# AniketRajpoot/DeepMusicGeneration

Hardware: NVIDIA B200
Metric: generated_tokens_per_sec (higher is better)
Workload: dtype bf16

## Files before the change

### deepmusicgeneration_b200/csrc/attention_decode2.cu

```cuda
#include "attention_decode3.cuh"

namespace dmg {

bool attn_decode2_supported(int Dh, int M) { return Dh == 64 && M >= 64 && M % 64 == 0 && d2_pick_groups(M) > 0; }

template <int G>
__global__ void __launch_bounds__((4 * G + 1) * 32, 1)
attn_decode2_kernel(const __grid_constant__ CUtensorMap tmK, const __grid_constant__ CUtensorMap tmV,
                    const __grid_constant__ CUtensorMap tmR, const AttnDecodeArgs a, int n_stages, int b0) {
  extern __shared__ __align__(1024) uint8_t d2_smem[];
  attn_decode2_body<G>(tmK, tmV, tmR, a, n_stages, b0, (int)blockIdx.x, (int)gridDim.x, d2_smem);
}

template <int G>
static int launch_d2(const TensorMap2D* tmK, const TensorMap2D* tmV, const TensorMap2D* tmR, const AttnDecodeArgs& a, int b0,
                     int num_sms, cudaStream_t st) {
  const int ns = d2_pick_stages(a.M, G);
  const D2Layout L = d2_layout(a.M, G, ns);
  static int configured = 0;
  if (configured < L.total) {
    DMG_CUDA_OK(cudaFuncSetAttribute(attn_decode2_kernel<G>, cudaFuncAttributeMaxDynamicSharedMemorySize, L.total));
    configured = L.total;
  }
  DMG_CHECK(ns >= 2, "attn_decode2: no stage count fits (M=%d)", a.M);
  const long long NI = (long long)a.B * a.H;
  const int grid = (int)(NI < num_sms ? NI : num_sms);
  return launch_k(attn_decode2_kernel<G>, dim3(grid), dim3((4 * G + 1) * 32), L.total, st, 1, *(const CUtensorMap*)tmK->bytes,
                  *(const CUtensorMap*)tmV->bytes, *(const CUtensorMap*)tmR->bytes, a, ns, b0);
}

bool attn_decode3_supported(int Dh, int M) { return Dh == 64 && M >= D3_KEYS && M <= 512 && M % D3_KEYS == 0 && d3_pick_stages(M) >= 2; }

__global__ void __launch_bounds__(D3_THREADS, 1)
attn_decode3_kernel(const __grid_constant__ CUtensorMap tmK, const __grid_constant__ CUtensorMap tmV,
                    const __grid_constant__ CUtensorMap tmR, const AttnDecodeArgs a, int n_stages, int b0) {
  extern __shared__ __align__(1024) uint8_t d3_smem[];
  attn_decode3_body<D3_TEAMS>(tmK, tmV, tmR, a, n_stages, b0, (int)blockIdx.x, (int)gridDim.x, d3_smem);
}

static int attn_decode3(const TensorMap2D* tmK, const TensorMap2D* tmV, const TensorMap2D* tmR, const AttnDecodeArgs& a_in, int b0,
                        int num_sms, cudaStream_t st) {
  const int ns = d3_pick_stages(a_in.M);
  const D3Layout L = d3_layout(a_in.M, ns);
  static int configured = 0;
  if (configured < L.total) {
    DMG_CUDA_OK(cudaFuncSetAttribute(attn_decode3_kernel, cudaFuncAttributeMaxDynamicSharedMemorySize, L.total));
    configured = L.total;
  }
  const int HD = a_in.H * 64;
  const int per = (int)((long long)D3_CAP * num_sms / a_in.H);
  DMG_CHECK(per >= 1, "attn_decode3: %d heads do not fit %d CTAs of %d items", a_in.H, num_sms, D3_CAP);
  for (int c0 = 0; c0 < a_in.B; c0 += per) {
    AttnDecodeArgs a = a_in;
    a.B = a_in.B - c0 < per ? a_in.B - c0 : per;
    a.qkv = a_in.qkv + (size_t)c0 * 3 * HD;
    a.out = a_in.out + (size_t)c0 * HD;
    a.kring = a_in.kring + (size_t)c0 * a_in.H * a_in.M * 64;
    a.vring = a_in.vring + (size_t)c0 * a_in.H * a_in.M * 64;
    const long long NI = (long long)a.B * a.H;
    const int grid = (int)(NI < num_sms ? NI : num_sms);
    if (launch_k(attn_decode3_kernel, dim3(grid), dim3(D3_THREADS), L.total, st, 1, *(const CUtensorMap*)tmK->bytes,
                 *(const CUtensorMap*)tmV->bytes, *(const CUtensorMap*)tmR->bytes, a, ns, b0 + c0)) return -1;
  }
  return 0;
}

int attn_decode2(const TensorMap2D* tmK, const TensorMap2D* tmV, const TensorMap2D* tmR, const AttnDecodeArgs& a_in, int b0,
                 int num_sms, cudaStream_t st) {
  static const int no_early = getenv("DMG_NO_EARLY_KV") ? 1 : 0;
  static const int env_v2 = getenv("DMG_ATTN_DECODE_V2") ? 1 : 0;
  AttnDecodeArgs a = a_in;
  a.no_early_kv = no_early;
  DMG_CHECK(a.Dcap >= a.M + 1, "attn_decode2: rel-pos cache too small (%d < %d)", a.Dcap, a.M + 1);
  if (!a.force_v2 && !env_v2 && attn_decode3_supported(64, a.M))
    return attn_decode3(tmK, tmV, tmR, a, b0, num_sms, st);
  const int G = d2_pick_groups(a.M);
  DMG_CHECK(G > 0, "attn_decode2: mem_len %d not supported", a.M);
  if (G == 4) return launch_d2<4>(tmK, tmV, tmR, a, b0, num_sms, st);
  if (G == 2) return launch_d2<2>(tmK, tmV, tmR, a, b0, num_sms, st);
  return launch_d2<1>(tmK, tmV, tmR, a, b0, num_sms, st);
}

}
```

### deepmusicgeneration_b200/csrc/attention_decode3.cuh

```cuda
#pragma once
#include "attention_decode2.cuh"

namespace dmg {

constexpr int D3_TEAMS = 2;
constexpr int D3_CAP = 16;
constexpr int D3_KEYS = 128;
constexpr int D3_TILE = D3_KEYS * 128;
constexpr int D3_THREADS = D3_TEAMS * 5 * 32;

struct D3Layout {
  int r_boxes, n_stages, tab_stride, free_bytes;
  int off_ring, off_r, off_tab, off_team, team_bytes, off_bar, total;
};

__host__ __device__ inline D3Layout d3_layout(int M, int n_stages, int teams = D3_TEAMS) {
  D3Layout L;
  L.r_boxes = (M + 1 + 63) / 64;
  L.n_stages = n_stages;
  L.tab_stride = M + 4;
  const int ring = teams * n_stages * D3_TILE;
  L.off_ring = 0;
  L.off_r = ring - L.r_boxes * 8192;
  L.free_bytes = L.off_r;
  L.off_tab = ring;
  L.off_team = L.off_tab + D3_CAP * L.tab_stride * 4;
  L.team_bytes = 2 * 768 + (((M + 16) * 2 + 15) & ~15) + 64;
  L.off_bar = (L.off_team + teams * L.team_bytes + 15) & ~15;
  L.total = L.off_bar + (teams * (2 * n_stages + 4) + 2) * 8 + 1024 ;
  return L;
}

static inline int d3_pick_stages(int M, int teams = D3_TEAMS) {
  for (int s = 6; s >= 2; s--) {
    const D3Layout L = d3_layout(M, s, teams);
    if (L.off_r >= 0 && L.total <= 227 * 1024) return s;
  }
  return 0;
}

template <int T>
__device__ __forceinline__ void attn_decode3_body(const CUtensorMap& tmK, const CUtensorMap& tmV, const CUtensorMap& tmR, const AttnDecodeArgs& a,
                                                  int n_stages, int b0, int cta, int ncta, uint8_t* d3_smem) {
  constexpr int CW = 4 * T;
  uint8_t* base = d3_smem + ((1024u - (smem_u32(d3_smem) & 1023u)) & 1023u);
  const int M = a.M, H = a.H, B = a.B, HD = H * 64;
  const D3Layout L = d3_layout(M, n_stages, T);
  uint8_t* Rres = base + L.off_r;
  float* tab = (float*)(base + L.off_tab);
  const int S = L.tab_stride;
  uint64_t* bars = (uint64_t*)(base + L.off_bar);
  uint64_t* r_full = bars;
  uint64_t* prologue_done = bars + 1;

  const int tid = threadIdx.x, warp = tid >> 5, lane = tid & 31;
  const int nT = M / D3_KEYS;
  pdl_launch_dependents();
  const long long NI = (long long)B * H;
  const int lo = (int)(NI * cta / ncta), hi = (int)(NI * (cta + 1) / ncta);
  const int n_items = hi - lo;

  if (tid == 0) {
    for (int t = 0; t < T; t++) {
      uint64_t* tb = bars + 2 + t * (2 * n_stages + 4);
      for (int s = 0; s < n_stages; s++) {
        mbar_init(&tb[s], 1);
        mbar_init(&tb[n_stages + s], 4);
      }
      for (int s = 0; s < 2; s++) {
        mbar_init(&tb[2 * n_stages + s], 1);
        mbar_init(&tb[2 * n_stages + 2 + s], 4);
      }
    }
    mbar_init(r_full, 1);
    mbar_init(prologue_done, CW);
    mbar_fence_init();
    tma_prefetch_desc(&tmK);
    tma_prefetch_desc(&tmV);
    tma_prefetch_desc(&tmR);
    if (n_items > 0) {
      mbar_expect_tx(r_full, (uint32_t)(L.r_boxes * 8192));
      for (int bx = 0; bx < L.r_boxes; bx++) tma_load_2d(Rres + bx * 8192, &tmR, 0, (lo / B) * a.Dcap + bx * 64, r_full);
    }
  }
  named_bar_sync(4, (CW + T) * 32);

  if (warp >= CW) {
    if (lane == 0) {
      const int team = warp - CW;
      uint64_t* tb = bars + 2 + team * (2 * n_stages + 4);
      uint64_t *full = tb, *empty = tb + n_stages, *q_full = tb + 2 * n_stages, *q_empty = q_full + 2;
      uint8_t* ring = base + L.off_ring;
      float* qbuf = (float*)(base + L.off_team + team * L.team_bytes);
      int s = 0, use = 0, pre = 0;
      bool alias_ok = false;
      const uint64_t kv_policy = l2_policy_evict_first();
      if (team < n_items && !a.no_early_kv) {
        const int it = lo + team, h = it / B, b = it - h * B;
        const int row0 = ((b0 + b) * H + h) * M;
        while (pre < 2 * nT && s < n_stages && (s * T + team + 1) * D3_TILE <= L.free_bytes) {
          mbar_expect_tx(&full[s], (uint32_t)D3_TILE);
          uint8_t* dst = ring + (s * T + team) * D3_TILE;
          const CUtensorMap* tm = pre < nT ? &tmK : &tmV;
          const int r0 = row0 + (pre < nT ? pre : pre - nT) * D3_KEYS;
          tma_load_2d_hint(dst, tm, 0, r0, &full[s], kv_policy);
          tma_load_2d_hint(dst + 8192, tm, 0, r0 + 64, &full[s], kv_policy);
          ++pre; ++s;
        }
        if (s == n_stages) { s = 0; use = 1; }
      }
      pdl_wait();
      for (int i = team, k = 0; i < n_items; i += T, ++k) {
        const int it = lo + i, h = it / B, b = it - h * B;
        const int qs = k & 1;
        mbar_wait(&q_empty[qs], (uint32_t)(((k >> 1) & 1) ^ 1));
        mbar_expect_tx(&q_full[qs], 768);
        const float* qrow = a.qkv + (size_t)b * 3 * HD + h * 64;
        bulk_g2s(qbuf + qs * 192, qrow, 256, &q_full[qs]);
        bulk_g2s(qbuf + qs * 192 + 64, qrow + HD, 256, &q_full[qs]);
        bulk_g2s(qbuf + qs * 192 + 128, qrow + 2 * HD, 256, &q_full[qs]);
        const int row0 = ((b0 + b) * H + h) * M;
        for (int t = (k == 0 ? pre : 0); t < 2 * nT; ++t) {
          if (!alias_ok && (s * T + team + 1) * D3_TILE > L.free_bytes) {
            mbar_wait(prologue_done, 0);
            alias_ok = true;
          }
          mbar_wait(&empty[s], (uint32_t)((use & 1) ^ 1));
          mbar_expect_tx(&full[s], (uint32_t)D3_TILE);
          uint8_t* dst = ring + (s * T + team) * D3_TILE;
          const CUtensorMap* tm = t < nT ? &tmK : &tmV;
          const int r0 = row0 + (t < nT ? t : t - nT) * D3_KEYS;
          tma_load_2d_hint(dst, tm, 0, r0, &full[s], kv_policy);
          tma_load_2d_hint(dst + 8192, tm, 0, r0 + 64, &full[s], kv_policy);
          if (++s == n_stages) { s = 0; ++use; }
        }
      }
    }
    return;
  }

  if (a.dbg && cta == 0 && tid == 0) { unsigned long long t; asm volatile("mov.u64 %0, %%globaltimer;" : "=l"(t)); a.dbg[48] = t; }
#ifdef D2_PROFILE
  long long prof[6] = {0, 0, 0, 0, 0, 0}, sec[8] = {0, 0, 0, 0, 0, 0, 0, 0};
  const long long t_begin = clock64();
  long long t_last = t_begin;
#endif
  pdl_wait();
  const int pos_total = a.dev_state[0], mc = a.dev_state[1];
  const int head = pos_total % M;
  const int team = warp >> 2, w = warp & 3;
  const int g = lane >> 2, t4 = lane & 3;
  const int hi16 = lane >> 4;
  const float sscale = a.scale * D2_LOG2E;

  {
    const uint32_t r_base = smem_u32(Rres);
    const int nblk = (M + 1 + 15) / 16;
    int seg = 0, r_epoch = 0;
    while (seg < n_items) {
      const int h = (lo + seg) / B;
      const int seg_end = min(n_items, (h + 1) * B - lo);
      mbar_wait(r_full, (uint32_t)(r_epoch & 1));
      r_epoch++;
      uint32_t qvf[2][4][2];
#pragma unroll
      for (int nb = 0; nb < 2; nb++) {
        const int item = min(seg + 8 * nb + g, seg_end - 1);
        const float* qrow = a.qkv + (size_t)(lo + item - h * B) * 3 * HD + h * 64;
#pragma unroll
        for (int ks = 0; ks < 4; ks++) {
#pragma unroll
          for (int hh = 0; hh < 2; hh++) {
            const int d = ks * 16 + 2 * t4 + 8 * hh;
            const float2 qq = *(const float2*)(qrow + d), vv = *(const float2*)(a.v + h * 64 + d);
            qvf[nb][ks][hh] = pack_bf16x2(qq.x + vv.x, qq.y + vv.y);
          }
        }
      }
      const bool two = seg_end - seg > 8;
      for (int blk = warp; blk < nblk; blk += CW) {
        const int dr = 16 * blk + (lane & 15);
        const uint32_t r_row = r_base + dr * 128;
        const int rsw = dr & 7;
        float acc0[4] = {0.f, 0.f, 0.f, 0.f}, acc1[4] = {0.f, 0.f, 0.f, 0.f};
#pragma unroll
        for (int ks = 0; ks < 4; ks++) {
          uint32_t c0, c1, c2, c3;
          ldmatrix_x4(r_row + (((2 * ks + hi16) ^ rsw) << 4), c0, c1, c2, c3);
          mma_bf16_16816(acc0, c0, c1, c2, c3, qvf[0][ks][0], qvf[0][ks][1]);
          if (two) mma_bf16_16816(acc1, c0, c1, c2, c3, qvf[1][ks][0], qvf[1][ks][1]);
        }
        const int d0 = 16 * blk + g, d1 = d0 + 8;
#pragma unroll
        for (int nb = 0; nb < 2; nb++) {
          const float* acc = nb ? acc1 : acc0;
          const int i0 = seg + 8 * nb + 2 * t4;
          if (i0 < seg_end) {
            if (d0 <= M) tab[i0 * S + d0] = acc[0];
            if (d1 <= M) tab[i0 * S + d1] = acc[2];
          }
          if (i0 + 1 < seg_end) {
            if (d0 <= M) tab[(i0 + 1) * S + d0] = acc[1];
            if (d1 <= M) tab[(i0 + 1) * S + d1] = acc[3];
          }
        }
      }
      seg = seg_end;
      named_bar_sync(5, CW * 32);
      if (seg < n_items && tid == 0) {
        mbar_expect_tx(r_full, (uint32_t)(L.r_boxes * 8192));
        for (int bx = 0; bx < L.r_boxes; bx++) tma_load_2d(Rres + bx * 8192, &tmR, 0, ((lo + seg) / B) * a.Dcap + bx * 64, r_full);
// ... 160 lines not shown
```

### deepmusicgeneration_b200/csrc/decode_layer.cu

```cuda
#include <cuda.h>

#include "attention_decode3.cuh"
#include "kernels.cuh"
#include "launch.cuh"

namespace dmg {
namespace {

constexpr int DL_STAGES = 10;
constexpr int DL_STAGE = 128 * 128;
constexpr int DL_B_BYTES = DL_ROWS * 128;
constexpr int DL_D = 512;
constexpr int DL_XA_BYTES = DL_ROWS * DL_D * 2;
constexpr int DL_HS_KB = 4;
constexpr int DL_HS_BYTES = DL_HS_KB * DL_B_BYTES;
constexpr int DL_OWN = DL_ROWS / DL_CLUSTER;
constexpr int DL_X1_BYTES = DL_OWN * DL_D * 4;
constexpr int DL_MMAW = 2;
constexpr int DL_THREADS = 32 * (1 + DL_MMAW + 8);
constexpr int DL_EPI0 = 32 * (1 + DL_MMAW);
constexpr int DL_EPI = 256;
constexpr int DL_LN_BYTES = 4 * DL_D * 4;
constexpr int DL_SMEM = DL_STAGES * DL_STAGE + DL_XA_BYTES + DL_HS_BYTES + DL_X1_BYTES + DL_LN_BYTES + 512  + 1024 ;
constexpr int DL_TMEM_COLS = 512;
constexpr int DL_CHAIN = DL_ROWS;
static_assert(DL_SMEM <= 227 * 1024, "decode_layer_kernel: shared memory budget");

__device__ __forceinline__ uint64_t dl_desc_sw128(uint32_t smem_addr) {
  return (uint64_t)((smem_addr & 0x3FFFFu) >> 4) | (1ull << 16) | (64ull << 32) | (1ull << 46) | (2ull << 61);
}
__host__ __device__ constexpr uint32_t dl_idesc(int M, int N) {
  return (1u << 4) | (1u << 7) | (1u << 10) | ((uint32_t)(N >> 3) << 17) | ((uint32_t)(M >> 4) << 24);
}
__device__ __forceinline__ uint32_t dl_cluster_ctarank() {
  uint32_t r;
  asm volatile("mov.u32 %0, %%cluster_ctarank;" : "=r"(r));
  return r;
}
__device__ __forceinline__ void dl_arrive() { asm volatile("barrier.cluster.arrive.release;" ::: "memory"); }
__device__ __forceinline__ void dl_wait() { asm volatile("barrier.cluster.wait.acquire;" ::: "memory"); }
__device__ __forceinline__ void dl_fence_async_all() { asm volatile("fence.proxy.async;" ::: "memory"); }
__device__ __forceinline__ void dl_fence_async_smem() { asm volatile("fence.proxy.async.shared::cta;" ::: "memory"); }

__device__ __forceinline__ void tmem_ld_32x16(uint32_t taddr, uint32_t (&r)[16]) {
  asm volatile(
      "tcgen05.ld.sync.aligned.32x32b.x16.b32 {%0,%1,%2,%3,%4,%5,%6,%7,%8,%9,%10,%11,%12,%13,%14,%15}, [%16];"
      : "=r"(r[0]), "=r"(r[1]), "=r"(r[2]), "=r"(r[3]), "=r"(r[4]), "=r"(r[5]), "=r"(r[6]), "=r"(r[7]), "=r"(r[8]),
        "=r"(r[9]), "=r"(r[10]), "=r"(r[11]), "=r"(r[12]), "=r"(r[13]), "=r"(r[14]), "=r"(r[15])
      : "r"(taddr)
      : "memory");
}
__device__ __forceinline__ void dl_spin(uint64_t* bar, uint32_t parity) {
  uint32_t n = 0;
  while (!mbar_try_wait(bar, parity))
    if (++n > (1u << 27)) __trap();
}
__device__ __forceinline__ float4 ldcg4(const float* p) { return __ldcg((const float4*)p); }
__device__ __forceinline__ void dl_mark(unsigned long long* dbg, int role, int mark) {
  if (dbg == nullptr) return;
  unsigned long long t;
  asm volatile("mov.u64 %0, %%globaltimer;" : "=l"(t));
  dbg[role * 16 + mark] = t;
}

__device__ __forceinline__ float dl_gelu(float x) {
  float t;
  asm("tanh.approx.f32 %0, %1;" : "=f"(t) : "f"(0.7978845608028654f * (x + 0.044715f * x * x * x)));
  return 0.5f * x * (1.f + t);
}

__device__ __forceinline__ void dl_layernorm(float (&z)[64], const float* __restrict__ w, const float* __restrict__ b, int t) {
  float s = 0.f;
#pragma unroll
  for (int i = 0; i < 64; i++) s += z[i];
  s += __shfl_xor_sync(0xffffffffu, s, 1); s += __shfl_xor_sync(0xffffffffu, s, 2); s += __shfl_xor_sync(0xffffffffu, s, 4);
  const float mean = s * (1.f / DL_D);
  float q = 0.f;
#pragma unroll
  for (int i = 0; i < 64; i++) { const float c = z[i] - mean; q += c * c; }
  q += __shfl_xor_sync(0xffffffffu, q, 1); q += __shfl_xor_sync(0xffffffffu, q, 2); q += __shfl_xor_sync(0xffffffffu, q, 4);
  const float rstd = rsqrtf(q * (1.f / DL_D) + 1e-5f);
#pragma unroll
  for (int kb = 0; kb < 8; kb++) {
    const int c = 64 * kb + 8 * t;
    const float4 w0 = *(const float4*)(w + c), w1 = *(const float4*)(w + c + 4);
    const float4 b0 = *(const float4*)(b + c), b1 = *(const float4*)(b + c + 4);
    float* v = z + 8 * kb;
    v[0] = (v[0] - mean) * rstd * w0.x + b0.x; v[1] = (v[1] - mean) * rstd * w0.y + b0.y;
    v[2] = (v[2] - mean) * rstd * w0.z + b0.z; v[3] = (v[3] - mean) * rstd * w0.w + b0.w;
    v[4] = (v[4] - mean) * rstd * w1.x + b1.x; v[5] = (v[5] - mean) * rstd * w1.y + b1.y;
    v[6] = (v[6] - mean) * rstd * w1.z + b1.z; v[7] = (v[7] - mean) * rstd * w1.w + b1.w;
  }
}
__device__ __forceinline__ void dl_store_xa(uint8_t* xa_s, const float (&z)[64], int r, int t) {
#pragma unroll
  for (int kb = 0; kb < 8; kb++) {
    const float* v = z + 8 * kb;
    *(uint4*)(xa_s + kb * DL_B_BYTES + r * 128 + ((t ^ (r & 7)) << 4)) =
        make_uint4(pack_bf16x2(v[0], v[1]), pack_bf16x2(v[2], v[3]), pack_bf16x2(v[4], v[5]), pack_bf16x2(v[6], v[7]));
  }
}

__device__ __forceinline__ void dl_gather(uint32_t taddr, int nacc, float (&out)[16]) {
  uint32_t r[16];
  tmem_ld_32x16(taddr, r);
  tmem_ld_wait();
#pragma unroll
  for (int i = 0; i < 16; i++) out[i] = __uint_as_float(r[i]);
  for (int c = 1; c < nacc; c++) {
    tmem_ld_32x16(taddr + c * DL_CHAIN, r);
    tmem_ld_wait();
#pragma unroll
    for (int i = 0; i < 16; i++) out[i] += __uint_as_float(r[i]);
  }
}

__device__ __forceinline__ uint32_t dl_mapa(uint32_t local_addr, uint32_t rank) {
  uint32_t r;
  asm volatile("mapa.shared::cluster.u32 %0, %1, %2;" : "=r"(r) : "r"(local_addr), "r"(rank));
  return r;
}
__device__ __forceinline__ void dl_st_cluster_v4(uint32_t addr, uint4 v) {
  asm volatile("st.shared::cluster.v4.b32 [%0], {%1, %2, %3, %4};" ::"r"(addr), "r"(v.x), "r"(v.y), "r"(v.z), "r"(v.w) : "memory");
}

__device__ __forceinline__ void decode_layer_body(const CUtensorMap& tmAttn, const CUtensorMap& tmWo, const CUtensorMap& tmW1,
                                                  const CUtensorMap& tmW2, const CUtensorMap& tmWq, const DecodeLayerArgs& a_in, int cluster,
                                                  uint8_t* dl_smem) {
  DecodeLayerArgs a = a_in;
  if (cluster != 0 || dl_cluster_ctarank() != 0) a.dbg = nullptr;
  uint8_t* tiles = dl_smem + ((1024u - (smem_u32(dl_smem) & 1023u)) & 1023u);
  uint8_t* xa_s = tiles + DL_STAGES * DL_STAGE;
  uint8_t* hs_s = xa_s + DL_XA_BYTES;
  float* x1_s = (float*)(hs_s + DL_HS_BYTES);
  float* ln_s = x1_s + DL_OWN * DL_D;
  uint64_t* full = (uint64_t*)(ln_s + 4 * DL_D);
  uint64_t* empty = full + DL_STAGES;
  uint64_t* tmem_full = empty + DL_STAGES;
  uint64_t* xa_ready = tmem_full + 4;
  uint64_t* hs_ready = xa_ready + 2;
  uint64_t* attn_full = hs_ready + 1;
  uint32_t* tmem_holder = (uint32_t*)(attn_full + 1);

  const int warp = threadIdx.x >> 5, lane = threadIdx.x & 31;
  const int crank = (int)dl_cluster_ctarank();
  const int row0 = a.row_base + cluster * DL_ROWS;
  const bool body = (a.mode & 1) != 0, next = (a.mode & 2) != 0;
  const int nkb_A = a.HD >> 6, nkb_d = DL_D >> 6;
  constexpr int nB = 2, nC = 4, nD = 2;
  const int fB = a.di / DL_CLUSTER, fD = a.n3 / DL_CLUSTER;
  const int nA_use = body ? nkb_A : 0, nB_use = body ? nB * nkb_d : 0, nC_use = body ? nC * DL_HS_KB : 0, nD_use = next ? nD * nkb_d : 0;
  pdl_launch_dependents();

  if (warp == 0 && lane == 0) {
    tma_prefetch_desc(&tmWo); tma_prefetch_desc(&tmW1); tma_prefetch_desc(&tmW2); tma_prefetch_desc(&tmWq); tma_prefetch_desc(&tmAttn);
  }
  if (warp == 1 && lane == 0) {
    for (int s = 0; s < DL_STAGES; s++) { mbar_init(&full[s], 1); mbar_init(&empty[s], 1); }
    for (int p = 0; p < 4; p++) mbar_init(&tmem_full[p], DL_MMAW);
    mbar_init(&xa_ready[0], DL_EPI); mbar_init(&xa_ready[1], DL_EPI); mbar_init(hs_ready, DL_EPI); mbar_init(attn_full, 1);
    mbar_fence_init();
  }
  if (warp == 1 + DL_MMAW) tmem_alloc<DL_TMEM_COLS>(tmem_holder);
  tc_fence_before();
  __syncthreads();
  tc_fence_after();
  const uint32_t tmem_base = *tmem_holder;

  if (warp == 0) {
    if (lane == 0) dl_mark(a.dbg, 0, 0);
    const int total = nA_use + nB_use + nC_use + nD_use;
    int bar_state = 0;
    const uint64_t w_policy = l2_policy_evict_last();
    for (int r = 0; r < total; r += 8) {
      if (body && bar_state == 0 && r >= nA_use) { dl_arrive(); bar_state = 1; }
      if (body && bar_state == 1 && r + 8 > nA_use + DL_STAGES) { dl_wait(); dl_arrive(); bar_state = 2; }
      if (body && bar_state == 2 && r >= nA_use + nB_use) { dl_wait(); dl_arrive(); bar_state = 3; }
      if (body && bar_state == 3 && r + 8 > nA_use + nB_use + nC_use + DL_STAGES) { dl_wait(); dl_arrive(); bar_state = 4; }
      const int i = r + lane;
      if (lane < 8 && i < total) {
        const int s = i % DL_STAGES;
        if (i >= DL_STAGES) dl_spin(&empty[s], (uint32_t)((i / DL_STAGES) - 1) & 1u);
        uint8_t* dst = tiles + s * DL_STAGE;
        const CUtensorMap* tm; int c0, frow, boxes;
        if (i < nA_use) { tm = &tmWo; c0 = i * 64; frow = 64 * crank; boxes = 1; }
        else if (i < nA_use + nB_use) { const int j = i - nA_use; tm = &tmW1; c0 = (j / nB) * 64; frow = fB * crank + 128 * (j % nB); boxes = 2; }
        else if (i < nA_use + nB_use + nC_use) { const int j = i - nA_use - nB_use; tm = &tmW2; c0 = fB * crank + (j / nC) * 64; frow = 128 * (j % nC); boxes = 2; }
        else { const int j = i - nA_use - nB_use - nC_use; tm = &tmWq; c0 = (j / nD) * 64; frow = fD * crank + 128 * (j % nD); boxes = (j % nD) == 0 ? 2 : 1; }
        mbar_expect_tx(&full[s], (uint32_t)(boxes * 64 * 128));
        tma_load_2d_hint(dst, tm, c0, frow, &full[s], w_policy);
        if (boxes == 2) tma_load_2d_hint(dst + 64 * 128, tm, c0, frow + 64, &full[s], w_policy);
      }
      if (r == 0 && body) {
        pdl_wait();
        if (lane == 0) mbar_expect_tx(attn_full, (uint32_t)(nkb_A * DL_B_BYTES));
        __syncwarp();
        if (lane < nkb_A) tma_load_2d(xa_s + lane * DL_B_BYTES, &tmAttn, lane * 64, row0, attn_full);
      }
      __syncwarp();
    }
    if (lane == 0) dl_mark(a.dbg, 0, 6);
    if (body) {
      if (bar_state == 0) { dl_arrive(); bar_state = 1; }
      if (bar_state == 1) { dl_wait(); dl_arrive(); bar_state = 2; }
      if (bar_state == 2) { dl_wait(); dl_arrive(); bar_state = 3; }
      if (bar_state == 3) { dl_wait(); dl_arrive(); bar_state = 4; }
      dl_wait();
    }
  } else if (warp <= DL_MMAW) {
    int it = 0;
    const int mine = warp - 1;
    const uint32_t xa_addr = smem_u32(xa_s), hs_addr = smem_u32(hs_s), tiles_addr = smem_u32(tiles);
    constexpr uint64_t DHI = (1ull << 16) | (64ull << 32) | (1ull << 46) | (2ull << 61);
    auto kblock = [&](int i, uint32_t col, uint32_t idesc, uint32_t b_addr, int kb, int kbx) {
      if ((i & (DL_MMAW - 1)) != mine) return;
      const int s = i % DL_STAGES;
      dl_spin(&full[s], (uint32_t)(i / DL_STAGES) & 1u);
      tc_fence_after();
      if (elect_one()) {
        const uint64_t da = DHI | (uint64_t)(((tiles_addr + s * DL_STAGE) & 0x3FFFFu) >> 4), db = DHI | (uint64_t)((b_addr & 0x3FFFFu) >> 4);
        const uint32_t d = tmem_base + col + (uint32_t)(((kb & kbx) << 2) * DL_CHAIN);
#pragma unroll
        for (int l = 0; l < 4; l++)
          umma_bf16(d + (uint32_t)(l * DL_CHAIN), da + (uint64_t)(2 * l), db + (uint64_t)(2 * l), idesc, kb > kbx ? 1u : 0u);
        umma_commit(&empty[s]);
      }
      __syncwarp();
    };
    constexpr uint32_t ID64 = dl_idesc(64, DL_ROWS), ID128 = dl_idesc(128, DL_ROWS);
    if (lane == 0 && mine == 0) dl_mark(a.dbg, 1, 0);
    if (body) {
      {
        dl_spin(attn_full, 0);
        tc_fence_after();
        for (int kb = 0; kb < nkb_A; kb++) kblock(it++, 0, ID64, xa_addr + kb * DL_B_BYTES, kb, 1);
        if (elect_one()) {
          dl_mark(a.dbg, 1, 1);
          umma_commit(&tmem_full[0]);
        }
      }
      __syncwarp();
      dl_arrive();
      dl_wait();
      dl_arrive();
      {
        dl_spin(&xa_ready[0], 0);
        tc_fence_after();
        if (lane == 0) dl_mark(a.dbg, 1, 2);
        for (int kb = 0; kb < nkb_d; kb++)
          for (int t = 0; t < nB; t++) kblock(it++, (uint32_t)(t * 4 * DL_CHAIN), ID128, xa_addr + kb * DL_B_BYTES, kb, 0);
        if (elect_one()) {
          dl_mark(a.dbg, 1, 3);
          umma_commit(&tmem_full[1]);
        }
        __syncwarp();
        dl_spin(hs_ready, 0);
        tc_fence_after();
        for (int kb = 0; kb < DL_HS_KB; kb++)
          for (int t = 0; t < nC; t++) kblock(it++, (uint32_t)(t * 4 * DL_CHAIN), ID128, hs_addr + kb * DL_B_BYTES, kb, 0);
        if (elect_one()) {
          dl_mark(a.dbg, 1, 5);
          umma_commit(&tmem_full[2]);
        }
      }
      __syncwarp();
      dl_wait();
      dl_arrive();
      dl_wait();
      dl_arrive();
      dl_wait();
      asm volatile("fence.proxy.async.shared::cta;" ::: "memory");
    }
    if (next) {
      if (!body) dl_spin(&xa_ready[1], 0);
      tc_fence_after();
      if (lane == 0) dl_mark(a.dbg, 1, 6);
      for (int kb = 0; kb < nkb_d; kb++) {
        kblock(it++, 0, ID128, xa_addr + kb * DL_B_BYTES, kb, 0);
        kblock(it++, (uint32_t)(4 * DL_CHAIN), ID64, xa_addr + kb * DL_B_BYTES, kb, 0);
      }
      if (elect_one()) {
        dl_mark(a.dbg, 1, 7);
        umma_commit(&tmem_full[3]);
      }
    }
    __syncwarp();
  } else {
    const int q = warp & 3;
    const int half = (warp - 1 - DL_MMAW) >> 2;
    const int te = threadIdx.x - DL_EPI0;
    const int r = te >> 3, t = te & 7;
    const int lr = te >> 6, lc = te & 63;
    const int row = row0 + r;
    const bool valid = row < a.B;
    const int erow0 = row0 + 16 * half;
    const uint32_t tq = tmem_base + ((uint32_t)(q * 32) << 16) + (uint32_t)(16 * half);
    float z[64];
    const bool mk = te == 0;
    if (body) {
      const float* src[4] = {a.ln1w, a.ln1b, a.ln2w, a.ln2b};
#pragma unroll
      for (int i = 0; i < 4; i++) *(float2*)(ln_s + i * DL_D + 2 * te) = __ldg((const float2*)(src[i] + 2 * te));
      asm volatile("bar.sync 1, 256;" ::: "memory");
    }
    if (mk) dl_mark(a.dbg, 2, 0);
    pdl_wait();
    if (mk) dl_mark(a.dbg, 2, 1);
    float rs[8] = {0.f, 0.f, 0.f, 0.f, 0.f, 0.f, 0.f, 0.f};
    if (body) {
      if (valid) {
        const float4 x0 = ldcg4(a.x32 + (size_t)row * DL_D + 64 * crank + 8 * t), x1 = ldcg4(a.x32 + (size_t)row * DL_D + 64 * crank + 8 * t + 4);
        rs[0] = x0.x; rs[1] = x0.y; rs[2] = x0.z; rs[3] = x0.w; rs[4] = x1.x; rs[5] = x1.y; rs[6] = x1.z; rs[7] = x1.w;
      }
    } else {
#pragma unroll
      for (int kb = 0; kb < 8; kb++) {
        float4 x0 = make_float4(0.f, 0.f, 0.f, 0.f), x1 = x0;
        if (valid) { x0 = ldcg4(a.x32 + (size_t)row * DL_D + 64 * kb + 8 * t); x1 = ldcg4(a.x32 + (size_t)row * DL_D + 64 * kb + 8 * t + 4); }
        float* v = z + 8 * kb;
        v[0] = x0.x; v[1] = x0.y; v[2] = x0.z; v[3] = x0.w; v[4] = x1.x; v[5] = x1.y; v[6] = x1.z; v[7] = x1.w;
      }
    }
    float acc[16];
    if (body) {
      mbar_wait(&tmem_full[0], 0);
      tc_fence_after();
      if (mk) dl_mark(a.dbg, 2, 2);
      dl_gather(tq, 4 * nkb_A < 8 ? 4 * nkb_A : 8, acc);
      float* T = (float*)hs_s;
      float4* stats = (float4*)(hs_s + DL_ROWS * 64 * 4);
      if (lane < 16) {
        const int fl = 16 * q + lane;
        const float bias = a.bo ? __ldg(a.bo + 64 * crank + fl) : 0.f;
#pragma unroll
        for (int rr = 0; rr < 16; rr++) T[(16 * half + rr) * 64 + fl] = acc[rr] + bias;
      }
      tc_fence_before();
      asm volatile("bar.sync 1, 256;" ::: "memory");
      if (mk) dl_mark(a.dbg, 2, 3);
      float v[8];
      {
        const float4 t0 = *(const float4*)(T + r * 64 + 8 * t), t1 = *(const float4*)(T + r * 64 + 8 * t + 4);
        v[0] = t0.x + rs[0]; v[1] = t0.y + rs[1]; v[2] = t0.z + rs[2]; v[3] = t0.w + rs[3];
        v[4] = t1.x + rs[4]; v[5] = t1.y + rs[5]; v[6] = t1.z + rs[6]; v[7] = t1.w + rs[7];
      }
      float s1 = 0.f;
#pragma unroll
      for (int i = 0; i < 8; i++) s1 += v[i];
      s1 += __shfl_xor_sync(0xffffffffu, s1, 1); s1 += __shfl_xor_sync(0xffffffffu, s1, 2); s1 += __shfl_xor_sync(0xffffffffu, s1, 4);
      const float mj = s1 * (1.f / 64.f);
      float s2 = 0.f;
#pragma unroll
      for (int i = 0; i < 8; i++) { const float c = v[i] - mj; s2 += c * c; }
      s2 += __shfl_xor_sync(0xffffffffu, s2, 1); s2 += __shfl_xor_sync(0xffffffffu, s2, 2); s2 += __shfl_xor_sync(0xffffffffu, s2, 4);
      {
        const uint32_t off = smem_u32(stats + crank * DL_ROWS + r);
        dl_st_cluster_v4(dl_mapa(off, (uint32_t)t), make_uint4(__float_as_uint(mj), __float_as_uint(s2), 0u, 0u));
      }
      dl_arrive();
      dl_wait();
      if (mk) dl_mark(a.dbg, 2, 4);
      {
        float ms[DL_CLUSTER], qs[DL_CLUSTER], mean = 0.f;
#pragma unroll
        for (int p = 0; p < DL_CLUSTER; p++) { const float4 st = stats[p * DL_ROWS + r]; ms[p] = st.x; qs[p] = st.y; mean += st.x; }
        mean *= (1.f / DL_CLUSTER);
        float m2 = 0.f;
#pragma unroll
        for (int p = 0; p < DL_CLUSTER; p++) { const float dm = ms[p] - mean; m2 += qs[p] + 64.f * dm * dm; }
        const float rstd = rsqrtf(m2 * (1.f / DL_D) + 1e-5f);
        const float* w = ln_s + 64 * crank + 8 * t;
        const float* bb = ln_s + DL_D + 64 * crank + 8 * t;
#pragma unroll
        for (int i = 0; i < 8; i++) v[i] = (v[i] - mean) * rstd * w[i] + bb[i];
      }
      {
        const uint32_t xoff = smem_u32(x1_s + (r & 3) * DL_D + 64 * crank + 8 * t);
        const uint32_t xo = dl_mapa(xoff, (uint32_t)(r >> 2));
        dl_st_cluster_v4(xo, make_uint4(__float_as_uint(v[0]), __float_as_uint(v[1]), __float_as_uint(v[2]), __float_as_uint(v[3])));
        dl_st_cluster_v4(xo + 16, make_uint4(__float_as_uint(v[4]), __float_as_uint(v[5]), __float_as_uint(v[6]), __float_as_uint(v[7])));
        const uint4 packed = make_uint4(pack_bf16x2(v[0], v[1]), pack_bf16x2(v[2], v[3]), pack_bf16x2(v[4], v[5]), pack_bf16x2(v[6], v[7]));
        const uint32_t off = smem_u32(xa_s) + (uint32_t)(crank * DL_B_BYTES + r * 128 + ((t ^ (r & 7)) << 4));
#pragma unroll
        for (int p = 0; p < DL_CLUSTER; p++) dl_st_cluster_v4(dl_mapa(off, (uint32_t)p), packed);
      }
      dl_arrive();
      dl_wait();
      asm volatile("fence.proxy.async.shared::cta;" ::: "memory");
      mbar_arrive(&xa_ready[0]);
      if (mk) dl_mark(a.dbg, 2, 5);
      mbar_wait(&tmem_full[1], 0);
      tc_fence_after();
      if (mk) dl_mark(a.dbg, 2, 6);
#pragma unroll
      for (int tt = 0; tt < nB; tt++) {
        dl_gather(tq + tt * 4 * DL_CHAIN, 4, acc);
        const int fl = 128 * tt + 32 * q + lane;
        const float bias = a.b1 ? __ldg(a.b1 + fB * crank + fl) : 0.f;
        uint8_t* base = hs_s + (fl >> 6) * DL_B_BYTES + (fl & 7) * 2;
        const int ch = (fl & 63) >> 3;
#pragma unroll
        for (int rr = 0; rr < 16; rr++) {
          const int rw = 16 * half + rr;
          *(bf16*)(base + rw * 128 + ((ch ^ (rw & 7)) << 4)) = __float2bfloat16_rn(dl_gelu(acc[rr] + bias));
        }
      }
      tc_fence_before();
      dl_fence_async_smem();
      mbar_arrive(hs_ready);
      if (mk) dl_mark(a.dbg, 2, 7);
      mbar_wait(&tmem_full[2], 0);
      tc_fence_after();
      if (mk) dl_mark(a.dbg, 2, 9);
      float* pp = a.PP + (size_t)crank * a.pp_stride;
#pragma unroll
      for (int tt = 0; tt < nC; tt++) {
        dl_gather(tq + tt * 4 * DL_CHAIN, 4, acc);
        const int f = 128 * tt + 32 * q + lane;
#pragma unroll
        for (int rr = 0; rr < 16; rr++) pp[(size_t)(erow0 + rr) * DL_D + f] = acc[rr];
      }
      tc_fence_before();
      __syncwarp();
      if (mk) dl_mark(a.dbg, 2, 10);
      dl_arrive();
      dl_wait();
      if (mk) dl_mark(a.dbg, 2, 11);
      {
        const int crow = DL_OWN * crank + lr;
        const int grow = row0 + crow;
        const int c0 = 8 * lc;
        float v[8];
        const float4 xa0 = *(const float4*)(x1_s + lr * DL_D + c0), xa1 = *(const float4*)(x1_s + lr * DL_D + c0 + 4);
        v[0] = xa0.x; v[1] = xa0.y; v[2] = xa0.z; v[3] = xa0.w; v[4] = xa1.x; v[5] = xa1.y; v[6] = xa1.z; v[7] = xa1.w;
        if (a.b2) {
          const float4 b0 = __ldg((const float4*)(a.b2 + c0)), b1 = __ldg((const float4*)(a.b2 + c0 + 4));
          v[0] += b0.x; v[1] += b0.y; v[2] += b0.z; v[3] += b0.w; v[4] += b1.x; v[5] += b1.y; v[6] += b1.z; v[7] += b1.w;
        }
#pragma unroll
        for (int p = 0; p < DL_CLUSTER; p++) {
          const float* src = a.PP + (size_t)p * a.pp_stride + (size_t)grow * DL_D + c0;
          const float4 p0 = ldcg4(src), p1 = ldcg4(src + 4);
          v[0] += p0.x; v[1] += p0.y; v[2] += p0.z; v[3] += p0.w; v[4] += p1.x; v[5] += p1.y; v[6] += p1.z; v[7] += p1.w;
        }
        float* red = (float*)(tmem_holder + 4);
        float s1 = 0.f;
#pragma unroll
        for (int i = 0; i < 8; i++) s1 += v[i];
        s1 = warp_sum(s1);
        if (lane == 0) red[(te >> 5)] = s1;
        asm volatile("bar.sync 1, 256;" ::: "memory");
        const float mean = (red[2 * lr] + red[2 * lr + 1]) * (1.f / DL_D);
        float s2 = 0.f;
#pragma unroll
        for (int i = 0; i < 8; i++) { const float c = v[i] - mean; s2 += c * c; }
        s2 = warp_sum(s2);
        if (lane == 0) red[8 + (te >> 5)] = s2;
        asm volatile("bar.sync 1, 256;" ::: "memory");
        const float rstd = rsqrtf((red[8 + 2 * lr] + red[8 + 2 * lr + 1]) * (1.f / DL_D) + 1e-5f);
        const float* w = ln_s + 2 * DL_D + c0;
        const float* bb = ln_s + 3 * DL_D + c0;
#pragma unroll
        for (int i = 0; i < 8; i++) v[i] = (v[i] - mean) * rstd * w[i] + bb[i];
        const uint4 packed = make_uint4(pack_bf16x2(v[0], v[1]), pack_bf16x2(v[2], v[3]), pack_bf16x2(v[4], v[5]), pack_bf16x2(v[6], v[7]));
        if (grow < a.B) {
          float* dst = a.x32 + (size_t)grow * DL_D + c0;
          *(float4*)dst = make_float4(v[0], v[1], v[2], v[3]);
          *(float4*)(dst + 4) = make_float4(v[4], v[5], v[6], v[7]);
          if (a.xa_out) *(uint4*)(a.xa_out + (size_t)grow * DL_D + c0) = packed;
        }
        if (next) {
          const uint32_t off = smem_u32(xa_s) + (uint32_t)((lc >> 3) * DL_B_BYTES + crow * 128 + (((lc & 7) ^ (crow & 7)) << 4));
#pragma unroll
          for (int p = 0; p < DL_CLUSTER; p++) dl_st_cluster_v4(dl_mapa(off, (uint32_t)p), packed);
        }
      }
      if (mk) dl_mark(a.dbg, 2, 12);
      dl_arrive();
      dl_wait();
    } else if (next) {
      dl_store_xa(xa_s, z, r, t);
      dl_fence_async_smem();
      mbar_arrive(&xa_ready[1]);
    }
    if (next) {
      mbar_wait(&tmem_full[3], 0);
      tc_fence_after();
      if (mk) dl_mark(a.dbg, 2, 13);
#pragma unroll
      for (int tt = 0; tt < nD; tt++) {
        dl_gather(tq + tt * 4 * DL_CHAIN, 4, acc);
        const bool h64 = tt == 1;
        const int f = fD * crank + (h64 ? 128 + 16 * q + lane : 32 * q + lane);
        if (!h64 || lane < 16) {
          const float bias = a.bq ? __ldg(a.bq + f) : 0.f;
#pragma unroll
          for (int rr = 0; rr < 16; rr++)
            if (erow0 + rr < a.B) a.qkv[(size_t)(erow0 + rr) * a.n3 + f] = acc[rr] + bias;
        }
      }
      tc_fence_before();
      if (mk) dl_mark(a.dbg, 2, 14);
    }
  }
  __syncthreads();
  if (warp == 1 + DL_MMAW) tmem_dealloc<DL_TMEM_COLS>(tmem_base);
}

__global__ void __launch_bounds__(DL_THREADS, 1)
decode_layer_kernel(const __grid_constant__ CUtensorMap tmAttn, const __grid_constant__ CUtensorMap tmWo,
                    const __grid_constant__ CUtensorMap tmW1, const __grid_constant__ CUtensorMap tmW2,
                    const __grid_constant__ CUtensorMap tmWq, const DecodeLayerArgs a) {
  extern __shared__ __align__(1024) uint8_t dyn_smem[];
  decode_layer_body(tmAttn, tmWo, tmW1, tmW2, tmWq, a, (int)blockIdx.x / DL_CLUSTER, dyn_smem);
}

static_assert(D3_THREADS <= DL_THREADS, "the attention role runs on the first D3_THREADS threads of the block");
__global__ void __launch_bounds__(DL_THREADS, 1)
decode_dual_kernel(const __grid_constant__ CUtensorMap tmAttn, const __grid_constant__ CUtensorMap tmWo,
                   const __grid_constant__ CUtensorMap tmW1, const __grid_constant__ CUtensorMap tmW2,
                   const __grid_constant__ CUtensorMap tmWq, const DecodeLayerArgs fa, const __grid_constant__ CUtensorMap tmK,
                   const __grid_constant__ CUtensorMap tmV, const __grid_constant__ CUtensorMap tmR, const AttnDecodeArgs aa, int n_stages,
                   int b0, int n_fused) {
  extern __shared__ __align__(1024) uint8_t dyn_smem[];
  const int cluster = (int)blockIdx.x / DL_CLUSTER;
  if (cluster < n_fused) {
    decode_layer_body(tmAttn, tmWo, tmW1, tmW2, tmWq, fa, cluster, dyn_smem);
  } else if (threadIdx.x < D3_THREADS) {
    attn_decode3_body<D3_TEAMS>(tmK, tmV, tmR, aa, n_stages, b0, (int)blockIdx.x - n_fused * DL_CLUSTER,
                                (int)gridDim.x - n_fused * DL_CLUSTER, dyn_smem);
  }
}

}

bool decode_layer_supported(int d, int HD, int di, int n3) {
  return d == DL_D && HD % 64 == 0 && HD >= 64 && HD <= DL_D && di == DL_CLUSTER * 64 * DL_HS_KB && n3 == DL_CLUSTER * 192;
}

int decode_layer(const TensorMap2D* tmAttn, const TensorMap2D* tmWo, const TensorMap2D* tmW1, const TensorMap2D* tmW2,
                 const TensorMap2D* tmWq, const DecodeLayerArgs& a, cudaStream_t st) {
  DMG_CHECK(decode_layer_supported(a.d, a.HD, a.di, a.n3), "decode_layer: geometry d=%d HD=%d di=%d n3=%d not supported", a.d, a.HD, a.di, a.n3);
  static bool configured = false;
  if (!configured) {
    DMG_CUDA_OK(cudaFuncSetAttribute(decode_layer_kernel, cudaFuncAttributeMaxDynamicSharedMemorySize, DL_SMEM));
    configured = true;
  }
  const int clusters = (a.B - a.row_base + DL_ROWS - 1) / DL_ROWS;
  if (clusters <= 0) return 0;
  return launch_k(decode_layer_kernel, dim3(clusters * DL_CLUSTER), dim3(DL_THREADS), (size_t)DL_SMEM, st, DL_CLUSTER,
                  *(const CUtensorMap*)tmAttn->bytes, *(const CUtensorMap*)tmWo->bytes, *(const CUtensorMap*)tmW1->bytes,
                  *(const CUtensorMap*)tmW2->bytes, *(const CUtensorMap*)tmWq->bytes, a);
}


bool decode_dual_supported(int M) { return attn_decode3_supported(64, M); }
int decode_dual_max_items(int attn_clusters) { return attn_clusters * DL_CLUSTER * D3_CAP; }

int decode_dual_max_clusters() {
  static int cached = -1;
  if (cached >= 0) return cached;
  cudaLaunchConfig_t cfg = {};
  cfg.gridDim = dim3(DL_CLUSTER * 32); cfg.blockDim = dim3(DL_THREADS); cfg.dynamicSmemBytes = 227 * 1024;
  cudaLaunchAttribute attr[1];
  attr[0].id = cudaLaunchAttributeClusterDimension;
  attr[0].val.clusterDim.x = DL_CLUSTER; attr[0].val.clusterDim.y = 1; attr[0].val.clusterDim.z = 1;
  cfg.attrs = attr; cfg.numAttrs = 1;
  int n = 0;
  if (cudaFuncSetAttribute(decode_dual_kernel, cudaFuncAttributeMaxDynamicSharedMemorySize, 227 * 1024) != cudaSuccess ||
      cudaOccupancyMaxActiveClusters(&n, decode_dual_kernel, &cfg) != cudaSuccess) {
    cudaGetLastError();
    n = 0;
  }
  cached = n;
  return cached;
}

int decode_dual(const TensorMap2D* tmAttn, const TensorMap2D* tmWo, const TensorMap2D* tmW1, const TensorMap2D* tmW2, const TensorMap2D* tmWq,
                const DecodeLayerArgs& fa, const TensorMap2D* tmK, const TensorMap2D* tmV, const TensorMap2D* tmR, const AttnDecodeArgs& aa,
                int b0, int attn_clusters, cudaStream_t st) {
  DMG_CHECK(decode_layer_supported(fa.d, fa.HD, fa.di, fa.n3) && decode_dual_supported(aa.M), "decode_dual: geometry not supported");
  DMG_CHECK(aa.Dcap >= aa.M + 1, "decode_dual: rel-pos cache too small (%d < %d)", aa.Dcap, aa.M + 1);
  DMG_CHECK((long long)aa.B * aa.H <= decode_dual_max_items(attn_clusters), "decode_dual: %d x %d items do not fit %d attention clusters",
            aa.B, aa.H, attn_clusters);
  const int ns = d3_pick_stages(aa.M);
  const D3Layout L = d3_layout(aa.M, ns);
  const int smem = L.total > DL_SMEM ? L.total : DL_SMEM;
  static int configured = 0;
  if (configured < smem) {
    DMG_CUDA_OK(cudaFuncSetAttribute(decode_dual_kernel, cudaFuncAttributeMaxDynamicSharedMemorySize, smem));
    configured = smem;
  }
  const int n_fused = (fa.B - fa.row_base + DL_ROWS - 1) / DL_ROWS;
  DMG_CHECK(n_fused >= 1 && attn_clusters >= 1, "decode_dual: empty role");
  return launch_k(decode_dual_kernel, dim3((n_fused + attn_clusters) * DL_CLUSTER), dim3(DL_THREADS), (size_t)smem, st, DL_CLUSTER,
                  *(const CUtensorMap*)tmAttn->bytes, *(const CUtensorMap*)tmWo->bytes, *(const CUtensorMap*)tmW1->bytes,
                  *(const CUtensorMap*)tmW2->bytes, *(const CUtensorMap*)tmWq->bytes, fa, *(const CUtensorMap*)tmK->bytes,
                  *(const CUtensorMap*)tmV->bytes, *(const CUtensorMap*)tmR->bytes, aa, ns, b0, n_fused);
}

}
```

Before: 289,200.

## Replace cluster barriers with st.async mbarrier signaling and size attention table per CTA

Cluster-wide store-then-barrier handoffs in the fused decode layer (LayerNorm stats, x1/xa broadcast, LN2 output) become st.async remote stores that complete transaction bytes on per-CTA mbarriers. Consumers spin on those mbarriers with cluster-scope acquire, so several full cluster barriers drop out of the producer and MMA loops. The TMEM gather now issues two loads before each wait. The attention decode smem layout sizes its score table by the actual items per CTA instead of a fixed cap, which can free space for more pipeline stages. The risk is subtle ordering bugs, since the expected-tx byte counts must match exactly what is stored.

```diff
diff --git a/deepmusicgeneration_b200/csrc/attention_decode2.cu b/deepmusicgeneration_b200/csrc/attention_decode2.cu
--- a/deepmusicgeneration_b200/csrc/attention_decode2.cu
+++ b/deepmusicgeneration_b200/csrc/attention_decode2.cu
@@ -40,13 +40,7 @@
 
 static int attn_decode3(const TensorMap2D* tmK, const TensorMap2D* tmV, const TensorMap2D* tmR, const AttnDecodeArgs& a_in, int b0,
                         int num_sms, cudaStream_t st) {
-  const int ns = d3_pick_stages(a_in.M);
-  const D3Layout L = d3_layout(a_in.M, ns);
   static int configured = 0;
-  if (configured < L.total) {
-    DMG_CUDA_OK(cudaFuncSetAttribute(attn_decode3_kernel, cudaFuncAttributeMaxDynamicSharedMemorySize, L.total));
-    configured = L.total;
-  }
   const int HD = a_in.H * 64;
   const int per = (int)((long long)D3_CAP * num_sms / a_in.H);
   DMG_CHECK(per >= 1, "attn_decode3: %d heads do not fit %d CTAs of %d items", a_in.H, num_sms, D3_CAP);
@@ -59,6 +53,12 @@
     a.vring = a_in.vring + (size_t)c0 * a_in.H * a_in.M * 64;
     const long long NI = (long long)a.B * a.H;
     const int grid = (int)(NI < num_sms ? NI : num_sms);
+    const int cap = d3_cap(NI, grid), ns = d3_pick_stages(a.M, cap);
+    const D3Layout L = d3_layout(a.M, ns, cap);
+    if (configured < L.total) {
+      DMG_CUDA_OK(cudaFuncSetAttribute(attn_decode3_kernel, cudaFuncAttributeMaxDynamicSharedMemorySize, L.total));
+      configured = L.total;
+    }
     if (launch_k(attn_decode3_kernel, dim3(grid), dim3(D3_THREADS), L.total, st, 1, *(const CUtensorMap*)tmK->bytes,
                  *(const CUtensorMap*)tmV->bytes, *(const CUtensorMap*)tmR->bytes, a, ns, b0 + c0)) return -1;
   }
diff --git a/deepmusicgeneration_b200/csrc/attention_decode3.cuh b/deepmusicgeneration_b200/csrc/attention_decode3.cuh
--- a/deepmusicgeneration_b200/csrc/attention_decode3.cuh
+++ b/deepmusicgeneration_b200/csrc/attention_decode3.cuh
@@ -14,7 +14,9 @@
   int off_ring, off_r, off_tab, off_team, team_bytes, off_bar, total;
 };
 
-__host__ __device__ inline D3Layout d3_layout(int M, int n_stages, int teams = D3_TEAMS) {
+__host__ __device__ inline int d3_cap(long long NI, int ncta) { return (int)((NI + ncta - 1) / ncta); }
+
+__host__ __device__ inline D3Layout d3_layout(int M, int n_stages, int cap, int teams = D3_TEAMS) {
   D3Layout L;
   L.r_boxes = (M + 1 + 63) / 64;
   L.n_stages = n_stages;
@@ -24,16 +26,16 @@
   L.off_r = ring - L.r_boxes * 8192;
   L.free_bytes = L.off_r;
   L.off_tab = ring;
-  L.off_team = L.off_tab + D3_CAP * L.tab_stride * 4;
+  L.off_team = L.off_tab + cap * L.tab_stride * 4;
   L.team_bytes = 2 * 768 + (((M + 16) * 2 + 15) & ~15) + 64;
   L.off_bar = (L.off_team + teams * L.team_bytes + 15) & ~15;
   L.total = L.off_bar + (teams * (2 * n_stages + 4) + 2) * 8 + 1024 ;
   return L;
 }
 
-static inline int d3_pick_stages(int M, int teams = D3_TEAMS) {
+static inline int d3_pick_stages(int M, int cap = D3_CAP, int teams = D3_TEAMS) {
   for (int s = 6; s >= 2; s--) {
-    const D3Layout L = d3_layout(M, s, teams);
+    const D3Layout L = d3_layout(M, s, cap, teams);
     if (L.off_r >= 0 && L.total <= 227 * 1024) return s;
   }
   return 0;
@@ -45,7 +47,8 @@
   constexpr int CW = 4 * T;
   uint8_t* base = d3_smem + ((1024u - (smem_u32(d3_smem) & 1023u)) & 1023u);
   const int M = a.M, H = a.H, B = a.B, HD = H * 64;
-  const D3Layout L = d3_layout(M, n_stages, T);
+  const long long NI = (long long)B * H;
+  const D3Layout L = d3_layout(M, n_stages, d3_cap(NI, ncta), T);
   uint8_t* Rres = base + L.off_r;
   float* tab = (float*)(base + L.off_tab);
   const int S = L.tab_stride;
@@ -56,7 +59,6 @@
   const int tid = threadIdx.x, warp = tid >> 5, lane = tid & 31;
   const int nT = M / D3_KEYS;
   pdl_launch_dependents();
-  const long long NI = (long long)B * H;
   const int lo = (int)(NI * cta / ncta), hi = (int)(NI * (cta + 1) / ncta);
   const int n_items = hi - lo;
 
diff --git a/deepmusicgeneration_b200/csrc/decode_layer.cu b/deepmusicgeneration_b200/csrc/decode_layer.cu
--- a/deepmusicgeneration_b200/csrc/decode_layer.cu
+++ b/deepmusicgeneration_b200/csrc/decode_layer.cu
@@ -38,6 +38,7 @@
   return r;
 }
 __device__ __forceinline__ void dl_arrive() { asm volatile("barrier.cluster.arrive.release;" ::: "memory"); }
+__device__ __forceinline__ void dl_arrive_relaxed() { asm volatile("barrier.cluster.arrive.relaxed;" ::: "memory"); }
 __device__ __forceinline__ void dl_wait() { asm volatile("barrier.cluster.wait.acquire;" ::: "memory"); }
 __device__ __forceinline__ void dl_fence_async_all() { asm volatile("fence.proxy.async;" ::: "memory"); }
 __device__ __forceinline__ void dl_fence_async_smem() { asm volatile("fence.proxy.async.shared::cta;" ::: "memory"); }
@@ -54,6 +55,20 @@
   uint32_t n = 0;
   while (!mbar_try_wait(bar, parity))
     if (++n > (1u << 27)) __trap();
+}
+__device__ __forceinline__ void dl_spin_cluster(uint64_t* bar, uint32_t parity) {
+  uint32_t n = 0, ok = 0;
+  while (true) {
+    asm volatile(
+        "{\n\t.reg .pred p;\n\t"
+        "mbarrier.try_wait.parity.acquire.cluster.shared::cta.b64 p, [%1], %2;\n\t"
+        "selp.u32 %0, 1, 0, p;\n\t}"
+        : "=r"(ok)
+        : "r"(smem_u32(bar)), "r"(parity)
+        : "memory");
+    if (ok) return;
+    if (++n > (1u << 27)) __trap();
+  }
 }
 __device__ __forceinline__ float4 ldcg4(const float* p) { return __ldcg((const float4*)p); }
 __device__ __forceinline__ void dl_mark(unsigned long long* dbg, int role, int mark) {
@@ -102,16 +117,13 @@
 }
 
 __device__ __forceinline__ void dl_gather(uint32_t taddr, int nacc, float (&out)[16]) {
-  uint32_t r[16];
-  tmem_ld_32x16(taddr, r);
-  tmem_ld_wait();
-#pragma unroll
-  for (int i = 0; i < 16; i++) out[i] = __uint_as_float(r[i]);
-  for (int c = 1; c < nacc; c++) {
-    tmem_ld_32x16(taddr + c * DL_CHAIN, r);
+  uint32_t r0[16], r1[16];
+  for (int c = 0; c < nacc; c += 2) {
+    tmem_ld_32x16(taddr + c * DL_CHAIN, r0);
+    tmem_ld_32x16(taddr + (c + 1) * DL_CHAIN, r1);
     tmem_ld_wait();
 #pragma unroll
-    for (int i = 0; i < 16; i++) out[i] += __uint_as_float(r[i]);
+    for (int i = 0; i < 16; i++) out[i] = (c == 0 ? __uint_as_float(r0[i]) : out[i] + __uint_as_float(r0[i])) + __uint_as_float(r1[i]);
   }
 }
 
@@ -120,8 +132,10 @@
   asm volatile("mapa.shared::cluster.u32 %0, %1, %2;" : "=r"(r) : "r"(local_addr), "r"(rank));
   return r;
 }
-__device__ __forceinline__ void dl_st_cluster_v4(uint32_t addr, uint4 v) {
-  asm volatile("st.shared::cluster.v4.b32 [%0], {%1, %2, %3, %4};" ::"r"(addr), "r"(v.x), "r"(v.y), "r"(v.z), "r"(v.w) : "memory");
+__device__ __forceinline__ void dl_st_async_v4(uint32_t local_addr, uint4 v, uint64_t* bar, uint32_t rank) {
+  asm volatile("st.async.shared::cluster.mbarrier::complete_tx::bytes.v4.b32 [%0], {%1, %2, %3, %4}, [%5];"
+               ::"r"(dl_mapa(local_addr, rank)), "r"(v.x), "r"(v.y), "r"(v.z), "r"(v.w), "r"(dl_mapa(smem_u32(bar), rank))
+               : "memory");
 }
 
 __device__ __forceinline__ void decode_layer_body(const CUtensorMap& tmAttn, const CUtensorMap& tmWo, const CUtensorMap& tmW1,
@@ -140,7 +154,9 @@
   uint64_t* xa_ready = tmem_full + 4;
   uint64_t* hs_ready = xa_ready + 2;
   uint64_t* attn_full = hs_ready + 1;
-  uint32_t* tmem_holder = (uint32_t*)(attn_full + 1);
+  uint64_t* stats_full = attn_full + 1;
+  uint64_t* ln2_full = stats_full + 1;
+  uint32_t* tmem_holder = (uint32_t*)(ln2_full + 1);
 
   const int warp = threadIdx.x >> 5, lane = threadIdx.x & 31;
   const int crank = (int)dl_cluster_ctarank();
@@ -158,7 +174,13 @@
   if (warp == 1 && lane == 0) {
     for (int s = 0; s < DL_STAGES; s++) { mbar_init(&full[s], 1); mbar_init(&empty[s], 1); }
     for (int p = 0; p < 4; p++) mbar_init(&tmem_full[p], DL_MMAW);
-    mbar_init(&xa_ready[0], DL_EPI); mbar_init(&xa_ready[1], DL_EPI); mbar_init(hs_ready, DL_EPI); mbar_init(attn_full, 1);
+    mbar_init(&xa_ready[0], 1); mbar_init(&xa_ready[1], DL_EPI); mbar_init(hs_ready, DL_EPI); mbar_init(attn_full, 1);
+    mbar_init(stats_full, 1); mbar_init(ln2_full, 1);
+    if (body) {
+      mbar_expect_tx(stats_full, DL_CLUSTER * DL_ROWS * 16);
+      mbar_expect_tx(&xa_ready[0], DL_XA_BYTES + DL_X1_BYTES);
+      if (next) mbar_expect_tx(ln2_full, DL_XA_BYTES);
+    }
     mbar_fence_init();
   }
   if (warp == 1 + DL_MMAW) tmem_alloc<DL_TMEM_COLS>(tmem_holder);
@@ -166,17 +188,15 @@
   __syncthreads();
   tc_fence_after();
   const uint32_t tmem_base = *tmem_holder;
+  if (body) dl_arrive_relaxed();
 
   if (warp == 0) {
     if (lane == 0) dl_mark(a.dbg, 0, 0);
     const int total = nA_use + nB_use + nC_use + nD_use;
-    int bar_state = 0;
+    bool arrived1 = false;
     const uint64_t w_policy = l2_policy_evict_last();
     for (int r = 0; r < total; r += 8) {
-      if (body && bar_state == 0 && r >= nA_use) { dl_arrive(); bar_state = 1; }
-      if (body && bar_state == 1 && r + 8 > nA_use + DL_STAGES) { dl_wait(); dl_arrive(); bar_state = 2; }
-      if (body && bar_state == 2 && r >= nA_use + nB_use) { dl_wait(); dl_arrive(); bar_state = 3; }
-      if (body && bar_state == 3 && r + 8 > nA_use + nB_use + nC_use + DL_STAGES) { dl_wait(); dl_arrive(); bar_state = 4; }
+      if (body && !arrived1 && r + 8 > nA_use + nB_use + nC_use + DL_STAGES) { dl_wait(); dl_arrive_relaxed(); arrived1 = true; }
       const int i = r + lane;
       if (lane < 8 && i < total) {
         const int s = i % DL_STAGES;
@@ -201,10 +221,7 @@
     }
     if (lane == 0) dl_mark(a.dbg, 0, 6);
     if (body) {
-      if (bar_state == 0) { dl_arrive(); bar_state = 1; }
-      if (bar_state == 1) { dl_wait(); dl_arrive(); bar_state = 2; }
-      if (bar_state == 2) { dl_wait(); dl_arrive(); bar_state = 3; }
-      if (bar_state == 3) { dl_wait(); dl_arrive(); bar_state = 4; }
+      if (!arrived1) { dl_wait(); dl_arrive_relaxed(); }
       dl_wait();
     }
   } else if (warp <= DL_MMAW) {
@@ -240,11 +257,9 @@
         }
       }
       __syncwarp();
-      dl_arrive();
-      dl_wait();
-      dl_arrive();
       {
-        dl_spin(&xa_ready[0], 0);
+        dl_spin_cluster(&xa_ready[0], 0);
+        dl_fence_async_smem();
         tc_fence_after();
         if (lane == 0) dl_mark(a.dbg, 1, 2);
         for (int kb = 0; kb < nkb_d; kb++)
@@ -265,11 +280,12 @@
       }
       __syncwarp();
       dl_wait();
-      dl_arrive();
+      dl_arrive_relaxed();
       dl_wait();
-      dl_arrive();
-      dl_wait();
-      asm volatile("fence.proxy.async.shared::cta;" ::: "memory");
+      if (next) {
+        dl_spin_cluster(ln2_full, 0);
+        dl_fence_async_smem();
+      }
     }
     if (next) {
       if (!body) dl_spin(&xa_ready[1], 0);
@@ -353,12 +369,9 @@
 #pragma unroll
       for (int i = 0; i < 8; i++) { const float c = v[i] - mj; s2 += c * c; }
       s2 += __shfl_xor_sync(0xffffffffu, s2, 1); s2 += __shfl_xor_sync(0xffffffffu, s2, 2); s2 += __shfl_xor_sync(0xffffffffu, s2, 4);
-      {
-        const uint32_t off = smem_u32(stats + crank * DL_ROWS + r);
-        dl_st_cluster_v4(dl_mapa(off, (uint32_t)t), make_uint4(__float_as_uint(mj), __float_as_uint(s2), 0u, 0u));
-      }
-      dl_arrive();
       dl_wait();
+      dl_st_async_v4(smem_u32(stats + crank * DL_ROWS + r), make_uint4(__float_as_uint(mj), __float_as_uint(s2), 0u, 0u), stats_full, (uint32_t)t);
+      dl_spin_cluster(stats_full, 0);
       if (mk) dl_mark(a.dbg, 2, 4);
       {
         float ms[DL_CLUSTER], qs[DL_CLUSTER], mean = 0.f;
@@ -376,18 +389,14 @@
       }
       {
         const uint32_t xoff = smem_u32(x1_s + (r & 3) * DL_D + 64 * crank + 8 * t);
-        const uint32_t xo = dl_mapa(xoff, (uint32_t)(r >> 2));
-        dl_st_cluster_v4(xo, make_uint4(__float_as_uint(v[0]), __float_as_uint(v[1]), __float_as_uint(v[2]), __float_as_uint(v[3])));
-        dl_st_cluster_v4(xo + 16, make_uint4(__float_as_uint(v[4]), __float_as_uint(v[5]), __float_as_uint(v[6]), __float_as_uint(v[7])));
+        const uint32_t owner = (uint32_t)(r >> 2);
+        dl_st_async_v4(xoff, make_uint4(__float_as_uint(v[0]), __float_as_uint(v[1]), __float_as_uint(v[2]), __float_as_uint(v[3])), &xa_ready[0], owner);
+        dl_st_async_v4(xoff + 16, make_uint4(__float_as_uint(v[4]), __float_as_uint(v[5]), __float_as_uint(v[6]), __float_as_uint(v[7])), &xa_ready[0], owner);
         const uint4 packed = make_uint4(pack_bf16x2(v[0], v[1]), pack_bf16x2(v[2], v[3]), pack_bf16x2(v[4], v[5]), pack_bf16x2(v[6], v[7]));
         const uint32_t off = smem_u32(xa_s) + (uint32_t)(crank * DL_B_BYTES + r * 128 + ((t ^ (r & 7)) << 4));
 #pragma unroll
-        for (int p = 0; p < DL_CLUSTER; p++) dl_st_cluster_v4(dl_mapa(off, (uint32_t)p), packed);
-      }
-      dl_arrive();
-      dl_wait();
-      asm volatile("fence.proxy.async.shared::cta;" ::: "memory");
-      mbar_arrive(&xa_ready[0]);
+        for (int p = 0; p < DL_CLUSTER; p++) dl_st_async_v4(off, packed, &xa_ready[0], (uint32_t)p);
+      }
       if (mk) dl_mark(a.dbg, 2, 5);
       mbar_wait(&tmem_full[1], 0);
       tc_fence_after();
@@ -426,6 +435,7 @@
       dl_arrive();
       dl_wait();
       if (mk) dl_mark(a.dbg, 2, 11);
+      dl_spin_cluster(&xa_ready[0], 0);
       {
         const int crow = DL_OWN * crank + lr;
         const int grow = row0 + crow;
@@ -463,21 +473,19 @@
 #pragma unroll
         for (int i = 0; i < 8; i++) v[i] = (v[i] - mean) * rstd * w[i] + bb[i];
         const uint4 packed = make_uint4(pack_bf16x2(v[0], v[1]), pack_bf16x2(v[2], v[3]), pack_bf16x2(v[4], v[5]), pack_bf16x2(v[6], v[7]));
+        if (next) {
+          const uint32_t off = smem_u32(xa_s) + (uint32_t)((lc >> 3) * DL_B_BYTES + crow * 128 + (((lc & 7) ^ (crow & 7)) << 4));
+#pragma unroll
+          for (int p = 0; p < DL_CLUSTER; p++) dl_st_async_v4(off, packed, ln2_full, (uint32_t)p);
+        }
         if (grow < a.B) {
           float* dst = a.x32 + (size_t)grow * DL_D + c0;
           *(float4*)dst = make_float4(v[0], v[1], v[2], v[3]);
           *(float4*)(dst + 4) = make_float4(v[4], v[5], v[6], v[7]);
           if (a.xa_out) *(uint4*)(a.xa_out + (size_t)grow * DL_D + c0) = packed;
         }
-        if (next) {
-          const uint32_t off = smem_u32(xa_s) + (uint32_t)((lc >> 3) * DL_B_BYTES + crow * 128 + (((lc & 7) ^ (crow & 7)) << 4));
-#pragma unroll
-          for (int p = 0; p < DL_CLUSTER; p++) dl_st_cluster_v4(dl_mapa(off, (uint32_t)p), packed);
-        }
       }
       if (mk) dl_mark(a.dbg, 2, 12);
-      dl_arrive();
-      dl_wait();
     } else if (next) {
       dl_store_xa(xa_s, z, r, t);
       dl_fence_async_smem();
@@ -583,8 +591,8 @@
   DMG_CHECK(aa.Dcap >= aa.M + 1, "decode_dual: rel-pos cache too small (%d < %d)", aa.Dcap, aa.M + 1);
   DMG_CHECK((long long)aa.B * aa.H <= decode_dual_max_items(attn_clusters), "decode_dual: %d x %d items do not fit %d attention clusters",
             aa.B, aa.H, attn_clusters);
-  const int ns = d3_pick_stages(aa.M);
-  const D3Layout L = d3_layout(aa.M, ns);
+  const int cap = d3_cap((long long)aa.B * aa.H, attn_clusters * DL_CLUSTER), ns = d3_pick_stages(aa.M, cap);
+  const D3Layout L = d3_layout(aa.M, ns, cap);
   const int smem = L.total > DL_SMEM ? L.total : DL_SMEM;
   static int configured = 0;
   if (configured < smem) {
```

Result: faster. 294,000, median of 6 (+1.7%).
